# alexandre01/deepsvg

Measured on AMD Instinct MI355X. Metric: SVG icons/sec (train step) hierarchical_ordered d=256, higher is better.
Workload: dtype bf16; 1 GPU; hierarchical_ordered (Hierarchical, use_vae=False) G=8 S=30 d_model=256 ff=512 H=8 L=4x4; full train step = forward + SVGLoss + backward + grad-clip 1.0 + AdamW; dropout 0.1; global_batch=512, batch_per_gpu=512, parallelism=dp1, hip_graph=True, encoder_layout=packed (valid tokens only, exact)

## Files before the change

### deepsvg_amd/csrc/ffn_bwd_gate.hip

```cpp
#include <stdlib.h>
#include "mfma_frag.h"
#include "../../include/dsvg.h"

namespace {

constexpr int GT = 64;
constexpr int W2_BYTES = 256 * 64 * 2;
constexpr int SLOT = (2 * 64 * 128 + 64 * 64) * 2;
constexpr int HP_OFF = 2 * 64 * 128 * 2;
constexpr int NSLOT = 4;
constexpr int W2_AT = (NSLOT - 1) * SLOT;
constexpr int LDS_BYTES = NSLOT * SLOT;
static_assert(LDS_BYTES <= 160 * 1024, "LDS budget of a CU");
static_assert(W2_BYTES <= SLOT, "the W2p image fits a slot");

__device__ __forceinline__ int sw256(int r) { return ((r & 3) << 2) | ((r >> 2) & 3); }
__device__ __forceinline__ int sw128(int r) { return ((r >> 1) & 1) << 2; }

__device__ __forceinline__ void dma5(const char* s0, const char* s1, const char* s2, const char* s3, const char* s4,
                                     uint32_t lds) {
    uint32_t keep;
    asm volatile(
        "s_mov_b32 %0, m0\n\t"
        "s_mov_b32 m0, %6\n\t"
        "s_nop 0\n\t"
        "global_load_lds_dwordx4 %1, off\n\t"
        "s_add_u32 m0, m0, 0x400\n\t"
        "s_nop 0\n\t"
        "global_load_lds_dwordx4 %2, off\n\t"
        "s_add_u32 m0, m0, 0x400\n\t"
        "s_nop 0\n\t"
        "global_load_lds_dwordx4 %3, off\n\t"
        "s_add_u32 m0, m0, 0x400\n\t"
        "s_nop 0\n\t"
        "global_load_lds_dwordx4 %4, off\n\t"
        "s_add_u32 m0, m0, 0x400\n\t"
        "s_nop 0\n\t"
        "global_load_lds_dwordx4 %5, off\n\t"
        "s_mov_b32 m0, %0"
        : "=&s"(keep)
        : "v"(s0), "v"(s1), "v"(s2), "v"(s3), "v"(s4), "s"(lds)
        : "memory", "scc");
}
__device__ __forceinline__ void dma4(const char* s0, const char* s1, const char* s2, const char* s3, uint32_t lds) {
    uint32_t keep;
    asm volatile(
        "s_mov_b32 %0, m0\n\t"
        "s_mov_b32 m0, %5\n\t"
        "s_nop 0\n\t"
        "global_load_lds_dwordx4 %1, off\n\t"
        "s_add_u32 m0, m0, 0x400\n\t"
        "s_nop 0\n\t"
        "global_load_lds_dwordx4 %2, off\n\t"
        "s_add_u32 m0, m0, 0x400\n\t"
        "s_nop 0\n\t"
        "global_load_lds_dwordx4 %3, off\n\t"
        "s_add_u32 m0, m0, 0x400\n\t"
        "s_nop 0\n\t"
        "global_load_lds_dwordx4 %4, off\n\t"
        "s_mov_b32 m0, %0"
        : "=&s"(keep)
        : "v"(s0), "v"(s1), "v"(s2), "v"(s3), "s"(lds)
        : "memory", "scc");
}

__device__ __forceinline__ bf16x8 ld_tr(const char* img, uint32_t off0, uint32_t off1) {
    Frag8 f;
    f.h[0] = __builtin_amdgcn_ds_read_tr16_b64_v4i16((shortx4 __attribute__((address_space(3)))*)(img + off0));
    f.h[1] = __builtin_amdgcn_ds_read_tr16_b64_v4i16((shortx4 __attribute__((address_space(3)))*)(img + off1));
    return f.v;
}

__device__ __forceinline__ bf16x8 zero_from(const bf16x8& v, int lim) {
    Frag8 f;
    f.v = v;
    uint32_t w[4] = {f.u.x, f.u.y, f.u.z, f.u.w};
#pragma unroll
    for (int e = 0; e < 4; ++e) w[e] = 2 * e >= lim ? 0u : (2 * e + 1 >= lim ? (w[e] & 0xffffu) : w[e]);
    f.u = make_uint4(w[0], w[1], w[2], w[3]);
    return f.v;
}

__device__ __forceinline__ float rowsum8(const bf16x8& f, float s) {
    typedef __bf16 bf16x2 __attribute__((ext_vector_type(2)));
    Frag8 t;
    t.v = f;
    const uint32_t w[4] = {t.u.x, t.u.y, t.u.z, t.u.w};
    const bf16x2 one = __builtin_bit_cast(bf16x2, 0x3f803f80u);
#pragma unroll
    for (int e = 0; e < 4; ++e) s = __builtin_amdgcn_fdot2_f32_bf16(__builtin_bit_cast(bf16x2, w[e]), one, s, false);
    return s;
}

__global__ __launch_bounds__(512, 1) void ffn_gate_dw2_kernel(const bf16_t* __restrict__ dym, const bf16_t* __restrict__ hp,
                                                               const bf16_t* __restrict__ w2p, float gate_scale,
                                                               bf16_t* __restrict__ dpre, int T, int k_chunk, int xcd_map,
                                                               float* __restrict__ part, int part_bf16) {
    extern __shared__ __attribute__((aligned(1024))) char lds[];
    const int bid = (int)blockIdx.x;
    int c, z;
    if (xcd_map) { const int local = bid >> 3; c = local & 7; z = (local >> 3) * 8 + (bid & 7); }
    else { c = bid & 7; z = bid >> 3; }
    const int row_begin = z * k_chunk;
    const int row_end = min(T, row_begin + k_chunk);
    const int n_tiles = row_end > row_begin ? (row_end - row_begin + GT - 1) / GT : 0;

    const int tid = threadIdx.x, lane = tid & 63;
    const int wave = __builtin_amdgcn_readfirstlane(tid >> 6);
    const int h = lane >> 5;
    const uint32_t lds0 = (uint32_t)(uintptr_t)DSVG_LDS_PTR(lds);

    const char* src[5];
    int srow[5];
    long long sld[5];
#pragma unroll
    for (int i = 0; i < 5; ++i) {
        const int P = wave * 5 + i;
        if (P < 32) {
            const int r = 4 * (P & 15) + (lane >> 4);
            const int ch = (lane & 15) ^ sw256(r);
            src[i] = (const char*)dym + (size_t)(128 * (P >> 4) + 8 * ch) * 2;
            srow[i] = r;
            sld[i] = 256 * 2;
        } else {
            const int r = 8 * (P - 32) + (lane >> 3);
            const int ch = (lane & 7) ^ sw128(r);
            src[i] = (const char*)hp + (size_t)(64 * c + 8 * ch) * 2;
            srow[i] = r;
            sld[i] = 512 * 2;
        }
    }
    auto issue = [&](int s) {
        const int r0 = row_begin + s * GT;
        const char* a[5];
#pragma unroll
        for (int i = 0; i < 5; ++i) a[i] = src[i] + (size_t)min(r0 + srow[i], T - 1) * sld[i];
        const uint32_t dst = __builtin_amdgcn_readfirstlane(lds0 + (uint32_t)(s % NSLOT) * SLOT + (uint32_t)wave * 5 * 1024);
        dma5(a[0], a[1], a[2], a[3], a[4], dst);
    };
    auto wait_tile = [&](int s) {
        const int ahead = min(NSLOT - 2, n_tiles - 1 - s);
        if (ahead >= 2) asm volatile("s_waitcnt vmcnt(10)" ::: "memory");
        else if (ahead == 1) asm volatile("s_waitcnt vmcnt(5)" ::: "memory");
        else asm volatile("s_waitcnt vmcnt(0)" ::: "memory");
    };
    static_assert(NSLOT == 4, "wait_tile counts for a 4-slot ring");

    const int g = lane >> 4, q = lane & 15, qq = q >> 2, pp = q & 3;
    const bool p1 = wave < 4;
    const int wm = (wave >> 1) & 1, wn = wave & 1;
    const int ww = wave & 3;
    const int trow = 8 * (g >> 1) + qq;
    const int pr = 32 * wm + (lane & 31);
    const uint32_t w2_off = (uint32_t)(trow * 128 + 16 * ((4 * wn + 2 * (g & 1) + (pp >> 1)) ^ sw128(trow)) + 8 * (pp & 1));
    uint32_t da_off[2][2], hb_off[2];
#pragma unroll
    for (int it = 0; it < 2; ++it)
#pragma unroll
        for (int sc = 0; sc < 2; ++sc) {
            const int r = trow + 4 * sc;
            const int ch = 8 * (ww & 1) + 4 * it + 2 * (g & 1) + (pp >> 1);
            da_off[it][sc] = (uint32_t)((ww >> 1) * 16384 + r * 256 + 16 * (ch ^ sw256(r)) + 8 * (pp & 1));
        }
#pragma unroll
    for (int jn = 0; jn < 2; ++jn)
        hb_off[jn] = (uint32_t)(HP_OFF + trow * 128 + 16 * ((4 * jn + 2 * (g & 1) + (pp >> 1)) ^ sw128(trow)) + 8 * (pp & 1));

    floatx16 acc00, acc01, acc10, acc11;
#pragma unroll
    for (int r = 0; r < 16; ++r) { acc00[r] = 0.f; acc01[r] = 0.f; acc10[r] = 0.f; acc11[r] = 0.f; }
    const bool do_rs = !p1 && c == 0;
    float rsa0 = 0.f, rsa1 = 0.f, rsb0 = 0.f, rsb1 = 0.f;

    Frag8 w2f[16];

    auto dpre_tile = [&](int s) {
        const char* slot = lds + (s % NSLOT) * SLOT;
        const int r0 = row_begin + s * GT;
        floatx16 acc;
#pragma unroll
        for (int r = 0; r < 16; ++r) acc[r] = 0.f;
#pragma unroll
        for (int kk = 0; kk < 16; ++kk) {
            Frag8 a;
            a.u = *reinterpret_cast<const uint4*>(slot + (kk >> 3) * 16384 + pr * 256 +
                                                  16 * ((2 * (kk & 7) + h) ^ sw256(pr)));
            acc = __builtin_amdgcn_mfma_f32_32x32x16_bf16(w2f[kk].v, a.v, acc, 0, 0, 0);
        }
        uint32_t x[4][4];
#pragma unroll
        for (int gq = 0; gq < 4; ++gq)
#pragma unroll
            for (int e = 0; e < 4; ++e) x[gq][e] = __float_as_uint(acc[4 * gq + e]);
#pragma unroll
        for (int e = 0; e < 4; ++e) {
            auto s01 = __builtin_amdgcn_permlane32_swap(x[0][e], x[1][e], false, false);
            auto s23 = __builtin_amdgcn_permlane32_swap(x[2][e], x[3][e], false, false);
            x[0][e] = s01[0]; x[1][e] = s01[1]; x[2][e] = s23[0]; x[3][e] = s23[1];
        }
#pragma unroll
        for (int e = 0; e < 4; ++e) {
            auto s02 = __builtin_amdgcn_permlane32_swap(x[0][e], x[2][e], false, false);
            auto s13 = __builtin_amdgcn_permlane32_swap(x[1][e], x[3][e], false, false);
            x[0][e] = s02[0]; x[2][e] = s02[1]; x[1][e] = s13[0]; x[3][e] = s13[1];
        }
        uint4 pk[2];
#pragma unroll
        for (int cb = 0; cb < 2; ++cb) {
            float v[8];
#pragma unroll
            for (int e = 0; e < 4; ++e) { v[e] = __uint_as_float(x[2 * cb][e]); v[4 + e] = __uint_as_float(x[2 * cb + 1][e]); }
            const uint4 gt = *reinterpret_cast<const uint4*>(slot + HP_OFF + pr * 128 +
                                                             16 * ((4 * wn + 2 * h + cb) ^ sw128(pr)));
            const uint32_t gw[4] = {gt.x, gt.y, gt.z, gt.w};
#pragma unroll
            for (int e = 0; e < 4; ++e) {
                const float g0 = __uint_as_float(gw[e] << 16), g1 = __uint_as_float(gw[e] & 0xffff0000u);
                v[2 * e] = g0 > 0.f ? v[2 * e] * gate_scale : 0.f;
                v[2 * e + 1] = g1 > 0.f ? v[2 * e + 1] * gate_scale : 0.f;
            }
            pk[cb] = make_uint4(f2bf_pk(v[0], v[1]), f2bf_pk(v[2], v[3]), f2bf_pk(v[4], v[5]), f2bf_pk(v[6], v[7]));
        }
        const int m = r0 + pr;
        if (m < row_end) {
            bf16_t* cp = dpre + (size_t)m * 512 + 64 * c + 32 * wn + 16 * h;
            *reinterpret_cast<uint4*>(cp) = pk[0];
            *reinterpret_cast<uint4*>(cp + 8) = pk[1];
        }
    };
    auto g2p_tile = [&](int s) {
        const char* slot = lds + (s % NSLOT) * SLOT;
        const int r0 = row_begin + s * GT;
        const bool ragged = r0 + GT > row_end;
#pragma unroll
        for (int kk = 0; kk < 4; ++kk) {
            bf16x8 a0 = ld_tr(slot, da_off[0][0] + kk * 4096, da_off[0][1] + kk * 4096);
            bf16x8 a1 = ld_tr(slot, da_off[1][0] + kk * 4096, da_off[1][1] + kk * 4096);
            const bf16x8 b0 = ld_tr(slot, hb_off[0] + kk * 2048, hb_off[0] + kk * 2048 + 512);
            const bf16x8 b1 = ld_tr(slot, hb_off[1] + kk * 2048, hb_off[1] + kk * 2048 + 512);
            if (ragged) {
                const int lim = row_end - (r0 + 16 * kk + 8 * h);
                a0 = zero_from(a0, lim);
                a1 = zero_from(a1, lim);
            }
            acc00 = __builtin_amdgcn_mfma_f32_32x32x16_bf16(b0, a0, acc00, 0, 0, 0);
            acc01 = __builtin_amdgcn_mfma_f32_32x32x16_bf16(b0, a1, acc01, 0, 0, 0);
            acc10 = __builtin_amdgcn_mfma_f32_32x32x16_bf16(b1, a0, acc10, 0, 0, 0);
            acc11 = __builtin_amdgcn_mfma_f32_32x32x16_bf16(b1, a1, acc11, 0, 0, 0);
            if (do_rs) {
                if (kk < 2) { rsa0 = rowsum8(a0, rsa0); rsa1 = rowsum8(a1, rsa1); }
                else { rsb0 = rowsum8(a0, rsb0); rsb1 = rowsum8(a1, rsb1); }
            }
        }
    };

    if (n_tiles > 0) {
        issue(0);
        const char* a[4];
#pragma unroll
        for (int i = 0; i < 4; ++i) {
            const int r = 8 * (wave * 4 + i) + (lane >> 3);
            const int ch = (lane & 7) ^ sw128(r);
            a[i] = (const char*)w2p + ((size_t)r * 512 + 64 * c + 8 * ch) * 2;
        }
        dma4(a[0], a[1], a[2], a[3], __builtin_amdgcn_readfirstlane(lds0 + W2_AT + (uint32_t)wave * 4 * 1024));
        for (int s = 1; s < NSLOT - 1 && s < n_tiles; ++s) issue(s);
        wait_tile(0);
        __builtin_amdgcn_s_barrier();
    }
    if (p1) {
        if (n_tiles > 0) {
#pragma unroll
            for (int kk = 0; kk < 16; ++kk) w2f[kk].v = ld_tr(lds + W2_AT, w2_off + kk * 2048, w2_off + kk * 2048 + 512);
            asm volatile("s_waitcnt lgkmcnt(0)" ::: "memory");
        }
        for (int s = 0; s < n_tiles; ++s) {
            wait_tile(s);
            __builtin_amdgcn_s_barrier();
            if (s + NSLOT - 1 < n_tiles) issue(s + NSLOT - 1);
            dpre_tile(s);
        }
        return;
    }
    for (int s = 0; s < n_tiles; ++s) {
        wait_tile(s);
        __builtin_amdgcn_s_barrier();
        if (s + NSLOT - 1 < n_tiles) issue(s + NSLOT - 1);
        g2p_tile(s);
    }

    const size_t slice = dsvg_splitk_slice(256, 512, true);
    float* my_part = part + (size_t)z * slice;
    const int mrow = 64 * ww + (lane & 31);
    const int ncol = 64 * c;
    auto put = [&](const floatx16& v, int jn, int im) {
        const int m = mrow + 32 * im;
#pragma unroll
        for (int gq = 0; gq < 4; ++gq) {
            const int n = ncol + 32 * jn + 8 * gq + 4 * h;
            *reinterpret_cast<float4*>(my_part + (size_t)m * 512 + n) = make_float4(v[4 * gq], v[4 * gq + 1], v[4 * gq + 2], v[4 * gq + 3]);
        }
    };
    auto put_bf16 = [&](const floatx16& v, int jn, int im) {
        const int m = mrow + 32 * im;
        bf16_t* base = reinterpret_cast<bf16_t*>(my_part);
#pragma unroll
        for (int gp = 0; gp < 2; ++gp) {
            const uint32_t a0 = f2bf_pk(v[8 * gp + 0], v[8 * gp + 1]), a1 = f2bf_pk(v[8 * gp + 2], v[8 * gp + 3]);
            const uint32_t b0 = f2bf_pk(v[8 * gp + 4], v[8 * gp + 5]), b1 = f2bf_pk(v[8 * gp + 6], v[8 * gp + 7]);
            auto s0 = __builtin_amdgcn_permlane32_swap(a0, b0, false, false);
            auto s1 = __builtin_amdgcn_permlane32_swap(a1, b1, false, false);
            const int n = ncol + 32 * jn + 16 * gp + 8 * h;
            *reinterpret_cast<uint4*>(base + (size_t)m * 512 + n) = make_uint4(s0[0], s1[0], s0[1], s1[1]);
        }
    };
    if (part_bf16) { put_bf16(acc00, 0, 0); put_bf16(acc01, 0, 1); put_bf16(acc10, 1, 0); put_bf16(acc11, 1, 1); }
    else { put(acc00, 0, 0); put(acc01, 0, 1); put(acc10, 1, 0); put(acc11, 1, 1); }
    if (do_rs) {
        rsa0 += __shfl_xor(rsa0, 32, 64);
        rsa1 += __shfl_xor(rsa1, 32, 64);
        rsb0 += __shfl_xor(rsb0, 32, 64);
        rsb1 += __shfl_xor(rsb1, 32, 64);
        if (h == 0) {
            float* rs = my_part + 256 * 512;
            rs[mrow] = rsa0 + rsb0;
            rs[mrow + 32] = rsa1 + rsb1;
        }
    }
}

}

extern "C" int dsvg_ffn_gate_dw2(const void* dym, const void* hp, const void* w2p, float gate_scale, void* dpre,
                                 int64_t rows, int32_t split_k, float* g2p, float* db2, float* workspace,
                                 int64_t workspace_bytes, void* stream) {
    DSVG_CHECK_ARG(dym && hp && w2p && dpre && g2p && db2 && workspace, "ffn_gate_dw2: null operand");
    DSVG_CHECK_ARG(rows > 0 && rows < (1ll << 30) && split_k > 1, "ffn_gate_dw2: bad rows %lld / split_k %d",
                   (long long)rows, split_k);
    DSVG_CHECK_ARG(workspace_bytes >= dsvg_gemm_workspace_bytes(256, 512, split_k), "ffn_gate_dw2: workspace too small");
    DSVG_CHECK_ARG(!(((uintptr_t)dym | (uintptr_t)hp | (uintptr_t)w2p | (uintptr_t)dpre | (uintptr_t)workspace) & 15),
                   "ffn_gate_dw2: operands must be 16-byte aligned");
    static const bool pbf_on = !(getenv("DSVG_SPLITK_BF16") && atoi(getenv("DSVG_SPLITK_BF16")) == 0);
    hipStream_t st = (hipStream_t)stream;
    const int T = (int)rows;
    const int k_chunk = ((T + split_k - 1) / split_k + 63) / 64 * 64;
    int nsplit = (T + k_chunk - 1) / k_chunk;
    if ((split_k % 8) == 0) nsplit = split_k;
    const int pbf = (pbf_on && (T % 64) == 0) ? 1 : 0;
    static bool once = false;
    if (!once) {
        (void)hipFuncSetAttribute((const void*)ffn_gate_dw2_kernel, hipFuncAttributeMaxDynamicSharedMemorySize, LDS_BYTES);
        once = true;
    }
    hipLaunchKernelGGL(ffn_gate_dw2_kernel, dim3(8 * nsplit), dim3(512), LDS_BYTES, st, (const bf16_t*)dym,
                       (const bf16_t*)hp, (const bf16_t*)w2p, gate_scale, (bf16_t*)dpre, T, k_chunk,
                       (nsplit % 8) == 0 ? 1 : 0, workspace, pbf);
    DSVG_LAUNCH_CHECK("ffn_gate_dw2");
    const int64_t mn = 256 * 512;
    const int64_t slice = (int64_t)dsvg_splitk_slice(256, 512, true);
    int rc = pbf ? dsvg_reduce_partials_mixed(workspace, nsplit, slice, mn, mn, g2p, 0, st)
                 : dsvg_reduce_partials_strided(workspace, nsplit, slice, mn, g2p, 0, st);
    if (rc) return rc;
    return dsvg_reduce_partials_strided(workspace + mn, nsplit, slice, 256, db2, 0, st);
}
```

### deepsvg_amd/functional.py

```python
import math
import contextlib
import functools
import os

import torch

from . import ops

FFN_MIN_ROWS = int(os.environ.get("DSVG_FFN_MIN_ROWS", "16384"))
ATTN_MIN_ROWS = int(os.environ.get("DSVG_ATTN_MIN_ROWS", "16384"))
FFN_GATE_DW2 = os.environ.get("DSVG_FFN_GATE_DW2", "1") != "0"

LN_BWD_MASKED = os.environ.get("DSVG_LN_BWD_MASKED", "1") != "0"
DEFER_MORE = os.environ.get("DSVG_DEFER_MORE", "1") != "0"
HEAD_KPAD = os.environ.get("DSVG_HEAD_KPAD", "1") != "0"
GS_STACK = os.environ.get("DSVG_GS_STACK", "1") != "0"
_ATTN_VALU = os.environ.get("DSVG_ATTN_VALU") is not None
_ATTN_MFMA_MIN_S = int(os.environ.get("DSVG_ATTN_MFMA_MIN_S", "2"))
GS_REMAINDER = int(os.environ.get("DSVG_GS_REMAINDER", "512"))
SEQ_ROUND = 2048
HEAD_FUSED = os.environ.get("DSVG_HEAD_FUSED", "0") != "0"

_NULL_CTX = contextlib.nullcontext()

class Runtime:

    def __init__(self, dtype=torch.float32, seed=None, store=None, training=False, defer=False):
        self.dtype = dtype
        self.defer = bool(defer)
        self.seed = seed
        self.store = store
        self.training = training
        self.masked = {}
        self.last_layer_gs = False
        self.stack_group = None
        self.path_stage = False
        self.cond_grad = {}

    def cond_grad_block(self, z, rows):
        if z is None or z.dim() != 2 or z.stride(1) != 1 or z.dtype != torch.bfloat16:
            return None
        w, ld = z.shape[1], z.stride(0)
        if ld <= w or ld % w or w % 8 or w > 512:
            return None
        i = (z.storage_offset() % ld) // w
        if (z.storage_offset() % ld) % w:
            return None
        base = z.data_ptr() - i * w * z.element_size()
        key = (base, rows, ld)
        buf = self.cond_grad.get(key)
        if buf is None:
            if len(self.cond_grad) > 8:
                self.cond_grad.clear()
            buf = self.cond_grad[key] = torch.empty((rows, ld), dtype=z.dtype, device=z.device)
        return buf[:, i * w:(i + 1) * w]

    def deferring(self):
        return ops.DEFER if self.defer else _NULL_CTX

    def stack_group_begin(self):
        if self.stack_group is None:
            ops.GROUP.__enter__()
            self.stack_group = []
        return self.stack_group

    def stack_group_end(self):
        if self.stack_group is not None:
            ops.GROUP.__exit__(None, None, None)
            self.stack_group = None

    def deferring_tables(self):
        return ops.DEFER if self.defer and DEFER_MORE else _NULL_CTX

    def grouping(self):
        return ops.GROUP

    def p(self, rate):
        return float(rate) if (self.training and rate > 0.0) else 0.0

    def w(self, param):
        if self.dtype == torch.float32:
            return param.detach()
        if self.store is not None:
            v = self.store.lp(param)
            if v is not None:
                return v
        return param.detach().to(self.dtype)

    def grad_out(self, param):
        if self.store is not None:
            v = self.store.grad_view(param)
            if v is not None:
                return v
        return torch.empty(param.shape, dtype=torch.float32, device=param.device)


def _wgrad_tag():
    return ops.tag_default("wgrad") if ops.PROFILE_ON else _NULL_CTX


def _wgrad(rt, param, dy, x, *, a_drop_p=0.0, a_drop_site=0):
    out = rt.grad_out(param)
    n_out, k_in = param.shape
    T = dy.shape[0]
    with rt.deferring(), _wgrad_tag():
        ops.gemm(dy, x, a_kc=False, b_kc=False, out=out.view(n_out, k_in), a_drop_p=a_drop_p, a_drop_site=a_drop_site,
                 seed=rt.seed, split_k=ops.split_k_for(n_out, k_in, T))
    return out


def _wbgrad(rt, weight, bias, dy, x, blocks=None, *, out=None, split=None, defer=True):
    if split is None:
        split = ops.split_k_for(*weight.shape, dy.shape[0], target_blocks=blocks)
    dw, db = out if out is not None else (rt.grad_out(weight), rt.grad_out(bias))
    with (rt.deferring() if defer else _NULL_CTX), _wgrad_tag():
        if split > 1:
            ops.gemm(dy, x, a_kc=False, b_kc=False, out=dw, split_k=split, rowsum=db)
        else:
            ops.gemm(dy, x, a_kc=False, b_kc=False, out=dw)
            ops.colsum(dy, out=db)
    return dw, db


def _group_blocks(w):
    return 8 * -(-w.shape[0] // 128) * -(-w.shape[1] // 128)


def _bgrad(rt, param, dy, *, drop_p=0.0, drop_site=0):
    out = rt.grad_out(param)
    with rt.deferring():
        ops.colsum(dy, out=out, drop_p=drop_p, drop_site=drop_site, seed=rt.seed)
    return out


def _hand_masked(rt, dx, dxm, p, site):
    if len(rt.masked) > 8:
        rt.masked.clear()
    rt.masked[dx.data_ptr()] = (dxm, p, site, dx._version)


def _take_masked(rt, dx, p, site, rows=None):
    hit = rt.masked.pop(dx.data_ptr(), None)
    if hit is None:
        return None
    dxm, hp, hsite, ver = hit
    n = dx.shape[0] if rows is None else rows
    if (hp != p or hsite != site or dxm.dtype != dx.dtype or dxm.shape[0] < n or dxm.shape[1:] != dx.shape[1:]
            or dx._version != ver):
        return None
    return dxm[:n]


def _aligned2d(t, mult):
    if t.dim() == 2 and t.stride(1) == 1 and t.stride(0) % mult == 0 and t.data_ptr() % 16 == 0:
        return t
    rows, cols = t.shape
    ld = (cols + mult - 1) // mult * mult
    buf = torch.zeros((rows, ld), dtype=t.dtype, device=t.device)
    buf[:, :cols].copy_(t)
    return buf[:, :cols]


class LinearFn(torch.autograd.Function):

# ... 456 lines not shown
        if _gs_eligible(rt, x, key_mask, n_seq, S, n_heads) and not causal and seq_off is None and l is None and live is None:
            gs = rt.store.gs(win)
        if gs is not None:
            g = (z if wg is None else ops.gemm(z, rt.w(wg), bias=bg.detach())) if z is not None else None
            with ops.tag("gs"):
                res = ops.gs_layer_fwd(x, gs[0], bin_.detach(), bo.detach(), b1.detach(), b2.detach(), n1w.detach(),
                                       n1b.detach(), n2w.detach(), n2b.detach(), key_mask, n_seq, S, scale, 1e-5, p, site0,
                                       rt.seed, seq_add=g, train=want_bwd)
            if want_bwd:
                x2, mean1, rstd1, xn1, qkv, ao, x1, mean2, rstd2, xn2, h = res
            else:
                x2, mean1, rstd1, xn1, qkv, ao, x1, mean2, rstd2, xn2, h = (res,) + (None,) * 10
            ctx.gs, ctx.ffn_fused, ctx.tiles, ctx.causal, ctx.live = True, False, None, False, None
            rt.last_layer_gs = True
            ctx.rt, ctx.n_seq, ctx.S, ctx.n_heads, ctx.p, ctx.site0, ctx.scale = rt, n_seq, S, n_heads, p, site0, scale
            ctx.save_for_backward(x, key_mask, z, l, mean1, rstd1, xn1, qkv, ao, x1, mean2, rstd2, xn2, h,
                                  n1w, n1b, win, bin_, wo, bo, n2w, n2b, w1, b1, w2, b2, wg, bg, wg2, bg2, seq_off)
            return x2
        att = None
        if (_attn_fused_eligible(rt, x, x.shape[0], key_mask, n_heads, causal) and S <= 32
                and (seq_off is None or tiles is not None) and p <= 0.5):
            att = rt.store.attn(win)
        z_fused = False
        split = 0
        if (att is not None and want_bwd and GS_REMAINDER > 0 and seq_off is None and key_mask is None and l is None
                and x.shape[0] == n_seq * S and x.shape[0] >= FFN_MIN_ROWS and n_seq > SEQ_ROUND):
            rem = n_seq % SEQ_ROUND
            if 0 < rem <= GS_REMAINDER and rt.store.gs(win) is not None and rt.store.ffn(w1) is not None:
                split = n_seq - rem
        if split:
            gsr, ffn = rt.store.gs(win), rt.store.ffn(w1)
            T, R0 = x.shape[0], split * S
            bf = lambda w_: torch.empty((T, w_), dtype=x.dtype, device=x.device)
            f32 = lambda n_: torch.empty(n_, dtype=torch.float32, device=x.device)
            x1, xn1, qkv, ao, mean1, rstd1 = bf(256), bf(256), bf(768), bf(256), f32(T), f32(T)
            x2, h, xn2 = bf(256), bf(512), bf(256)
            g = None
            if z is not None:
                g = z if wg is None else ops.gemm(z, rt.w(wg), bias=bg.detach())
                z_fused = True
            with ops.tag("attn"):
                ops.attn_block_fwd(x[:R0], att, bin_.detach(), bo.detach(), n1w.detach(), n1b.detach(), None, split, S, scale,
                                   1e-5, p, site0, site0 + 1, rt.seed, train=True, seq_add=None if g is None else g[:split],
                                   site_seq_add=site0 + 2,
                                   into=(x1[:R0], xn1[:R0], qkv[:R0], ao[:R0], mean1[:R0], rstd1[:R0]))
            with ops.tag("ffn"):
                ops.ffn_fwd(x1[:R0], ffn[0], ffn[2], b2.detach(), 1e-5, p, site0 + 3, site0 + 4, rt.seed, out=x2[:R0],
                            train=True, into=(h[:R0], xn2[:R0]))
            with ops.tag("gs"):
                ops.gs_layer_fwd(x[R0:], gsr[0], bin_.detach(), bo.detach(), b1.detach(), b2.detach(), n1w.detach(),
                                 n1b.detach(), n2w.detach(), n2b.detach(), None, n_seq - split, S, scale, 1e-5, p, site0,
                                 rt.seed, seq_add=None if g is None else g[split:], train=True, seq_base=split, ffn_format=True,
                                 into=(x2[R0:], mean1[R0:], rstd1[R0:], xn1[R0:], qkv[R0:], ao[R0:], x1[R0:], f32(T - R0),
                                       f32(T - R0), xn2[R0:], h[R0:]))
            mean2 = rstd2 = None
        elif att is not None:
            g = None
            if z is not None and seq_off is None and x.shape[0] == n_seq * S:
                g = z if wg is None else ops.gemm(z, rt.w(wg), bias=bg.detach())
                z_fused = True
            with ops.tag("attn"):
                res = ops.attn_block_fwd(x, att, bin_.detach(), bo.detach(), n1w.detach(), n1b.detach(), key_mask, n_seq,
                                         S, scale, 1e-5, p, site0, site0 + 1, rt.seed, seq_off=seq_off, tiles=tiles,
                                         train=want_bwd, seq_add=g, site_seq_add=site0 + 2)
            if want_bwd:
                x1, xn1, qkv, ao, mean1, rstd1 = res
            else:
                x1, xn1, qkv, ao, mean1, rstd1 = res, None, None, None, None, None
        else:
            xn1, mean1, rstd1 = ops.layernorm_fwd(x, n1w.detach(), n1b.detach())
            qkv = ops.gemm(xn1, rt.w(win), bias=bin_.detach())
            if causal:
                ao = ops.attention_fwd(qkv, key_mask, n_seq, S, n_heads, scale, p, site0, rt.seed, causal=True)
            else:
                ao = ops.attention_fwd(qkv, key_mask, n_seq, S, n_heads, scale, p, site0, rt.seed, seq_off=seq_off,
                                       tiles=tiles, **_path_kw(rt, S))
            x1 = ops.gemm(ao, rt.w(wo), bias=bo.detach(), res=x, drop_p=p, drop_site=site0 + 1, seed=rt.seed)
        ctx.tiles, ctx.causal = tiles, causal
        if z is not None and not z_fused:
            g = z.contiguous() if wg is None else ops.gemm(z, rt.w(wg), bias=bg.detach())
            ops.bcast_add_fwd_(x1, g, n_seq, S, p, site0 + 2, rt.seed)
        if l is not None:
            g2 = ops.gemm(l, rt.w(wg2), bias=bg2.detach())
            ops.bcast_add_fwd_(x1, g2, n_seq, S, p, site0 + 5, rt.seed)
        ffn = rt.store.ffn(w1) if (rt.store is not None and x.dtype == torch.bfloat16 and x.shape[0] >= FFN_MIN_ROWS) else None
        ctx.ffn_fused = ffn is not None
        if split:
            pass
        elif ffn is not None:
            mean2 = rstd2 = None
            with ops.tag("ffn"):
                if want_bwd:
                    x2, h, xn2, _rstd = ops.ffn_fwd(x1, ffn[0], ffn[2], b2.detach(), 1e-5, p, site0 + 3, site0 + 4, rt.seed,
                                                    train=True)
                else:
                    xn2 = h = None
                    x2 = ops.ffn_fwd(x1, ffn[0], ffn[2], b2.detach(), 1e-5, p, site0 + 3, site0 + 4, rt.seed)
        else:
            with ops.tag("ffn"):
                xn2, mean2, rstd2 = ops.layernorm_fwd(x1, n2w.detach(), n2b.detach())
                h = ops.gemm(xn2, rt.w(w1), bias=b1.detach(), act=ops.RELU, drop_p=p, drop_site=site0 + 3, seed=rt.seed)
                x2 = ops.gemm(h, rt.w(w2), bias=b2.detach(), res=x1, drop_p=p, drop_site=site0 + 4, seed=rt.seed)
        ctx.rt, ctx.n_seq, ctx.S, ctx.n_heads, ctx.p, ctx.site0, ctx.scale = rt, n_seq, S, n_heads, p, site0, scale
        assert seq_off is None or (z is None and l is None), "packed layout: no per-sequence conditioning adds"
        ctx.live = _live_rows(live, x.shape[0])
        assert ctx.live is None or (seq_off is None and key_mask is None and l is None)
        ctx.save_for_backward(x, key_mask, z, l, mean1, rstd1, xn1, qkv, ao, x1, mean2, rstd2, xn2, h,
                              n1w, n1b, win, bin_, wo, bo, n2w, n2b, w1, b1, w2, b2, wg, bg, wg2, bg2, seq_off)
        return x2

    @staticmethod
    def backward(ctx, dx2):
        rt, n_seq, S, H, p, s0 = ctx.rt, ctx.n_seq, ctx.S, ctx.n_heads, ctx.p, ctx.site0
        (x, key_mask, z, l, mean1, rstd1, xn1, qkv, ao, x1, mean2, rstd2, xn2, h,
         n1w, n1b, win, bin_, wo, bo, n2w, n2b, w1, b1, w2, b2, wg, bg, wg2, bg2, seq_off) = ctx.saved_tensors
        dx2 = dx2.contiguous()
        full_rows, n_seq_full = x.shape[0], n_seq
        live = _armed(ctx.live)
        dx2_masked = _take_masked(rt, dx2, p, s0 + 4, rows=(live[1] if live is not None else None)) if p > 0 else None
        if live is not None:
            n_seq, R = live
            (dx2, x, mean1, rstd1, xn1, qkv, ao, x1, mean2, rstd2, xn2, h) = (
                (t[:R] if t is not None else None) for t in (dx2, x, mean1, rstd1, xn1, qkv, ao, x1, mean2, rstd2, xn2, h))
        inv_keep = ops.keep_scale(p)
        dx1m = None
        if ctx.gs:
            gs = rt.store.gs(win)
            with rt.deferring(), ops.tag("gs"):
                (dx, dx1, dym, dpre, dx1m, dqkv, dn2w, dn2b, dn1w, dn1b, *dg_) = ops.gs_layer_bwd(
                    dx2, gs[1], x, mean1, rstd1, qkv, x1, mean2, rstd2, h, n1w.detach(), n2w.detach(), key_mask, n_seq, S,
                    ctx.scale, p, s0, rt.seed, want_dx1=False, dgamma2=rt.grad_out(n2w),
                    dbeta2=rt.grad_out(n2b), dgamma1=rt.grad_out(n1w), dbeta1=rt.grad_out(n1b), want_dg=z is not None)
            dz = dg = None
            if z is not None:
                dg = dg_[0]
                if wg is None:
                    dz = dg
                elif ctx.needs_input_grad[3]:
                    dz = ops.gemm(dg, rt.w(wg), b_kc=False)
            (dw2, db2), (dw1, db1), (dwo, dbo), (dwin, dbin), (dwg, dbg) = _gs_queue_wgrads(
                rt, ctx.first_in_stack, (w2, b2, dym, h), (w1, b1, dpre, xn2), (wo, bo, dx1m, ao), (win, bin_, dqkv, xn1),
                cond=(wg if z is not None else None, bg, dg, z))
            return (None, dx, None, dz, None, None, None, None, None, None,
                    dn1w, dn1b, dwin, dbin, dwo, dbo, dn2w, dn2b, dw1, db1, dw2, db2, dwg, dbg, None, None, None, None, None,
                    None, None, None)
        if ctx.ffn_fused:
            pb, _b1f, w2p = rt.store.ffn(w1)[1:]
            T = x1.shape[0]
            with ops.tag("ffn"):
                g2p = torch.empty((256, 512), dtype=torch.float32, device=x1.device)
                g1p = torch.empty((512, 256), dtype=torch.float32, device=x1.device)
                db1p = torch.empty(512, dtype=torch.float32, device=x1.device)
                db2 = rt.grad_out(b2)
                s2, s1 = ops.split_k_for(256, 512, T), ops.split_k_for(512, 256, T)
                hp, xh = h, xn2
                dym = dx2_masked if dx2_masked is not None else ops.drop_apply(dx2, p, s0 + 4, rt.seed)
                if (FFN_GATE_DW2 and s2 > 1 and dym.is_cuda and dym.dtype == torch.bfloat16
                        and dym.is_contiguous() and hp.is_contiguous() and w2p.is_contiguous()):
                    with rt.deferring():
                        dpre = ops.ffn_gate_dw2(dym, hp, w2p, inv_keep, g2p, db2, s2)
                else:
                    _wbgrad(rt, None, None, dym, hp, out=(g2p, db2), split=s2)
                    dpre = ops.gemm(dym, w2p, b_kc=False, gate=hp, gate_scale=inv_keep)
                _wbgrad(rt, None, None, dpre, xh, out=(g1p, db1p), split=s1)
                dx1 = ops.ffn_bwd_dx(dpre, x1, dx2, pb)
                dw1, db1, dw2 = rt.grad_out(w1), rt.grad_out(b1), rt.grad_out(w2)
                dn2w, dn2b = rt.grad_out(n2w), rt.grad_out(n2b)
                fin = (g1p, db1p, g2p, w1.detach(), n2w.detach(), n2b.detach(), dw1.detach(), db1.detach(), dw2.detach(),
                       dn2w.detach(), dn2b.detach())
                if rt.defer:
                    ops.ffn_wgrad_finish_deferred(*fin)
                else:
                    ops.ffn_wgrad_finish(*fin)
            del hp, dpre, xh, dym
        else:
            with ops.tag("ffn"):
                dx2m = dx2_masked if dx2_masked is not None else ops.drop_apply(dx2, p, s0 + 4, rt.seed)
                dw2, db2 = _wbgrad(rt, w2, b2, dx2m, h)
                dh = ops.gemm(dx2m, rt.w(w2), b_kc=False, gate=h, gate_scale=inv_keep)
                dw1, db1 = _wbgrad(rt, w1, b1, dh, xn2)
                dxn2 = ops.gemm(dh, rt.w(w1), b_kc=False)
                with rt.deferring():
                    dx1, dn2w, dn2b = ops.layernorm_bwd(dxn2, x1, mean2, rstd2, n2w.detach(), res=dx2,
                                                        dgamma=rt.grad_out(n2w), dbeta=rt.grad_out(n2b))
            del dx2m
        dz = dl = dwg = dbg = dwg2 = dbg2 = None
        if l is not None:
            dg2 = ops.bcast_add_bwd(dx1, n_seq, S, p, s0 + 5, rt.seed)
            dwg2, dbg2 = _wbgrad(rt, wg2, bg2, dg2, l)
            if ctx.needs_input_grad[4]:
                dl = ops.gemm(dg2, rt.w(wg2), b_kc=False)
        if z is not None:
            vec = dx1.dtype == torch.bfloat16 and dx1.is_contiguous() and dx1.shape[1] % 8 == 0 and dx1.shape[1] <= 512
            dg_out = rt.cond_grad_block(z, n_seq_full) if (wg is None and vec and dx1.data_ptr() % 16 == 0) else None
            if p > 0 and vec and n_seq * S <= dx1.shape[0] <= n_seq_full * S:
                dg, dx1m = ops.bcast_add_bwd(dx1, n_seq, S, p, s0 + 2, rt.seed, n_seq_out=n_seq_full, mask_site=s0 + 1, out=dg_out)
            else:
                dg = ops.bcast_add_bwd(dx1, n_seq, S, p, s0 + 2, rt.seed, n_seq_out=n_seq_full, out=dg_out)
            if wg is None:
                dz = dg
            else:
                dwg, dbg = _wbgrad(rt, wg, bg, dg, z)
                if ctx.needs_input_grad[3]:
                    dz = ops.gemm(dg, rt.w(wg), b_kc=False)
        if dx1m is None:
            dx1m = ops.drop_apply(dx1, p, s0 + 1, rt.seed)
        dwo, dbo = _wbgrad(rt, wo, bo, dx1m, ao)
        wob = None
        if (not _ATTN_VALU and S >= _ATTN_MFMA_MIN_S and _attn_fused_eligible(rt, x, x.shape[0], key_mask, H, ctx.causal)
                and ((seq_off is None and 16 < S <= 32 and x.shape[0] >= n_seq * S) or (seq_off is not None and ctx.tiles is not None))):
            wob = rt.store.attn_bwd(win)
        if wob is not None:
            dqkv = ops.attention_bwd_outproj(qkv, key_mask, dx1m, wob, n_seq, S, ctx.scale, p, s0, rt.seed, seq_off=seq_off,
                                             tiles=ctx.tiles)
        else:
            dao = ops.gemm(dx1m, rt.w(wo), b_kc=False)
            if ctx.causal:
                dqkv = ops.attention_bwd(qkv, key_mask, dao, n_seq, S, H, ctx.scale, p, s0, rt.seed, causal=True)
            else:
                dqkv = ops.attention_bwd(qkv, key_mask, dao, n_seq, S, H, ctx.scale, p, s0, rt.seed, seq_off=seq_off,
                                         tiles=ctx.tiles, **_path_kw(rt, S))
        del dx1m
        dwin, dbin = _wbgrad(rt, win, bin_, dqkv, xn1)
        dx_out = None
        if live is not None:
            dx_full = torch.empty((full_rows, x.shape[1]), dtype=x.dtype, device=x.device)
            dx_out = dx_full[:x.shape[0]]
        mk = (p, ctx.mask_below, rt.seed) if (ctx.mask_below is not None and p > 0) else None
        with rt.deferring():
            dxn1 = ops.gemm(dqkv, rt.w(win), b_kc=False)
            out = ops.layernorm_bwd(dxn1, x, mean1, rstd1, n1w.detach(), res=dx1, dx=dx_out,
                                    dgamma=rt.grad_out(n1w), dbeta=rt.grad_out(n1b), masked=mk)
            dx, dn1w, dn1b = out[:3]
        if live is not None:
            dx = dx_full
        if mk is not None:
            _hand_masked(rt, dx, out[3], p, ctx.mask_below)
        return (None, dx, None, dz, dl, None, None, None, None, None,
                dn1w, dn1b, dwin, dbin, dwo, dbo, dn2w, dn2b, dw1, db1, dw2, db2, dwg, dbg, dwg2, dbg2, None, None, None,
                None, None, None)


def gs_stack_eligible(rt, x, key_mask, n_seq, S, n_heads, n_layers, wins):
    return (GS_STACK and x.dim() == 2 and _gs_eligible(rt, x, key_mask, n_seq, S, n_heads)
            and 1 <= n_layers <= ops.GS_STACK_MAX and all(rt.store.gs(w) is not None for w in wins))


class GsStackFn(torch.autograd.Function):

    @staticmethod
    def forward(ctx, rt, x, key_mask, n_seq, S, n_heads, drop_rate, site0, n_layers, has_g, *tensors):
        p = rt.p(drop_rate)
        per = 13 if has_g else 12
        assert len(tensors) == per * n_layers
        scale = float(x.shape[1] // n_heads) ** -0.5
        want_bwd = any(ctx.needs_input_grad)
        layers = []
        for i in range(n_layers):
            n1w, n1b, win, bin_, wo, bo, n2w, n2b, w1, b1, w2, b2 = tensors[per * i:per * i + 12]
            layers.append(dict(img=rt.store.gs(win)[0], in_bias=bin_.detach(), out_bias=bo.detach(), b1=b1.detach(), b2=b2.detach(),
                               gamma1=n1w.detach(), beta1=n1b.detach(), gamma2=n2w.detach(), beta2=n2b.detach(),
                               site0=site0 + 8 * i, seq_add=tensors[per * i + 12] if has_g else None))
        with ops.tag("gs"):
            res = ops.gs_stack_fwd(x, layers, key_mask, n_seq, S, scale, 1e-5, p, rt.seed, train=want_bwd)
        rt.last_layer_gs = True
        ctx.rt, ctx.n_seq, ctx.S, ctx.p, ctx.site0, ctx.scale, ctx.n, ctx.has_g = rt, n_seq, S, p, site0, scale, n_layers, has_g
        if not want_bwd:
            return res[-1]
        saved = [x, key_mask]
        for r in res:
            saved += list(r)
        ctx.save_for_backward(*saved, *tensors)
        return res[-1][0]

    @staticmethod
    def backward(ctx, dx2):
        rt, n_seq, S, p, n, has_g = ctx.rt, ctx.n_seq, ctx.S, ctx.p, ctx.n, ctx.has_g
        sv = ctx.saved_tensors
        x, key_mask = sv[0], sv[1]
        acts = [sv[2 + 11 * i:2 + 11 * (i + 1)] for i in range(n)]
        tensors = sv[2 + 11 * n:]
        per = 13 if has_g else 12
        prm = [tensors[per * i:per * i + 12] for i in range(n)]
        layers = []
        for i in range(n):
            x2, mean1, rstd1, xn1, qkv, ao, x1, mean2, rstd2, xn2, h = acts[i]
            n1w, n1b, win, bin_, wo, bo, n2w, n2b, w1, b1, w2, b2 = prm[i]
            layers.append(dict(img=rt.store.gs(win)[1], x=x if i == 0 else acts[i - 1][0], mean1=mean1, rstd1=rstd1, qkv=qkv, x1=x1,
                               mean2=mean2, rstd2=rstd2, h=h, gamma1=n1w.detach(), gamma2=n2w.detach(), site0=ctx.site0 + 8 * i,
                               dgamma2=rt.grad_out(n2w), dbeta2=rt.grad_out(n2b), dgamma1=rt.grad_out(n1w),
                               dbeta1=rt.grad_out(n1b)))
        with rt.deferring(), ops.tag("gs"):
            dx, ops_, dgcat = ops.gs_stack_bwd(dx2.contiguous(), layers, key_mask, n_seq, S, ctx.scale, p, rt.seed, want_dg=has_g)
        grads = [None] * (per * n)
        for i in range(n - 1, -1, -1):
            x2, mean1, rstd1, xn1, qkv, ao, x1, mean2, rstd2, xn2, h = acts[i]
            n1w, n1b, win, bin_, wo, bo, n2w, n2b, w1, b1, w2, b2 = prm[i]
            dym, dpre, dx1m, dqkv = ops_[i]
            (dw2, db2), (dw1, db1), (dwo, dbo), (dwin, dbin), _ = _gs_queue_wgrads(
                rt, i == 0, (w2, b2, dym, h), (w1, b1, dpre, xn2), (wo, bo, dx1m, ao), (win, bin_, dqkv, xn1))
            L = layers[i]
            grads[per * i:per * i + 12] = [L["dgamma1"], L["dbeta1"], dwin, dbin, dwo, dbo, L["dgamma2"], L["dbeta2"], dw1, db1, dw2, db2]
            if has_g:
                grads[per * i + 12] = dgcat[:, 256 * i:256 * (i + 1)]
        return (None, dx, None, None, None, None, None, None, None, None, *grads)


# ... 153 lines not shown
```

Baseline: 92040 icons/s.

## Widen gate/dW2 kernel column tile to 128 and double split-k

The fused FFN backward gate plus dW2 kernel now gives each block 128 hidden columns instead of 64, so only 4 column blocks are launched per k-chunk. It holds a larger W2 image that spans two LDS slots and uses a 3-slot ring with 6 DMA pieces per wave. The dpre path issues two MFMAs per loaded W2 fragment, and the dW2 path keeps 8 accumulators. This cuts redundant reloads of dym across column blocks and raises MFMA work per LDS byte. To keep the grid occupied, the split-k count targets twice as many blocks. The cost is a shallower prefetch pipeline, more registers, more partials to reduce, and an extra barrier before the second tile can be issued.

```diff
diff --git a/deepsvg_amd/csrc/ffn_bwd_gate.hip b/deepsvg_amd/csrc/ffn_bwd_gate.hip
--- a/deepsvg_amd/csrc/ffn_bwd_gate.hip
+++ b/deepsvg_amd/csrc/ffn_bwd_gate.hip
@@ -5,24 +5,26 @@
 namespace {
 
 constexpr int GT = 64;
-constexpr int W2_BYTES = 256 * 64 * 2;
-constexpr int SLOT = (2 * 64 * 128 + 64 * 64) * 2;
-constexpr int HP_OFF = 2 * 64 * 128 * 2;
-constexpr int NSLOT = 4;
-constexpr int W2_AT = (NSLOT - 1) * SLOT;
+constexpr int IMG = 64 * 128 * 2;
+constexpr int W2_BYTES = 4 * IMG;
+constexpr int SLOT = 3 * IMG;
+constexpr int HP_OFF = 2 * IMG;
+constexpr int NSLOT = 3;
+constexpr int PIECES = SLOT / 1024 / 8;
+constexpr int W2_AT = SLOT;
 constexpr int LDS_BYTES = NSLOT * SLOT;
 static_assert(LDS_BYTES <= 160 * 1024, "LDS budget of a CU");
-static_assert(W2_BYTES <= SLOT, "the W2p image fits a slot");
+static_assert(W2_AT + W2_BYTES <= LDS_BYTES, "the W2p image fits slots 1-2");
+static_assert(PIECES == 6, "dma6 / wait_tile count 6 pieces per wave and tile");
 
 __device__ __forceinline__ int sw256(int r) { return ((r & 3) << 2) | ((r >> 2) & 3); }
-__device__ __forceinline__ int sw128(int r) { return ((r >> 1) & 1) << 2; }
-
-__device__ __forceinline__ void dma5(const char* s0, const char* s1, const char* s2, const char* s3, const char* s4,
-                                     uint32_t lds) {
+
+__device__ __forceinline__ void dma6(const char* s0, const char* s1, const char* s2, const char* s3, const char* s4,
+                                     const char* s5, uint32_t lds) {
     uint32_t keep;
     asm volatile(
         "s_mov_b32 %0, m0\n\t"
-        "s_mov_b32 m0, %6\n\t"
+        "s_mov_b32 m0, %7\n\t"
         "s_nop 0\n\t"
         "global_load_lds_dwordx4 %1, off\n\t"
         "s_add_u32 m0, m0, 0x400\n\t"
@@ -37,9 +39,12 @@
         "s_add_u32 m0, m0, 0x400\n\t"
         "s_nop 0\n\t"
         "global_load_lds_dwordx4 %5, off\n\t"
+        "s_add_u32 m0, m0, 0x400\n\t"
+        "s_nop 0\n\t"
+        "global_load_lds_dwordx4 %6, off\n\t"
         "s_mov_b32 m0, %0"
         : "=&s"(keep)
-        : "v"(s0), "v"(s1), "v"(s2), "v"(s3), "v"(s4), "s"(lds)
+        : "v"(s0), "v"(s1), "v"(s2), "v"(s3), "v"(s4), "v"(s5), "s"(lds)
         : "memory", "scc");
 }
 __device__ __forceinline__ void dma4(const char* s0, const char* s1, const char* s2, const char* s3, uint32_t lds) {
@@ -99,8 +104,8 @@
     extern __shared__ __attribute__((aligned(1024))) char lds[];
     const int bid = (int)blockIdx.x;
     int c, z;
-    if (xcd_map) { const int local = bid >> 3; c = local & 7; z = (local >> 3) * 8 + (bid & 7); }
-    else { c = bid & 7; z = bid >> 3; }
+    if (xcd_map) { const int local = bid >> 3; c = local & 3; z = (local >> 2) * 8 + (bid & 7); }
+    else { c = bid & 3; z = bid >> 2; }
     const int row_begin = z * k_chunk;
     const int row_end = min(T, row_begin + k_chunk);
     const int n_tiles = row_end > row_begin ? (row_end - row_begin + GT - 1) / GT : 0;
@@ -110,88 +115,75 @@
     const int h = lane >> 5;
     const uint32_t lds0 = (uint32_t)(uintptr_t)DSVG_LDS_PTR(lds);
 
-    const char* src[5];
-    int srow[5];
-    long long sld[5];
-#pragma unroll
-    for (int i = 0; i < 5; ++i) {
-        const int P = wave * 5 + i;
+    const char* src[PIECES];
+    int srow[PIECES];
+    long long sld[PIECES];
+#pragma unroll
+    for (int i = 0; i < PIECES; ++i) {
+        const int P = wave * PIECES + i;
+        const int r = 4 * (P & 15) + (lane >> 4);
+        const int ch = (lane & 15) ^ sw256(r);
+        srow[i] = r;
         if (P < 32) {
-            const int r = 4 * (P & 15) + (lane >> 4);
-            const int ch = (lane & 15) ^ sw256(r);
             src[i] = (const char*)dym + (size_t)(128 * (P >> 4) + 8 * ch) * 2;
-            srow[i] = r;
             sld[i] = 256 * 2;
         } else {
-            const int r = 8 * (P - 32) + (lane >> 3);
-            const int ch = (lane & 7) ^ sw128(r);
-            src[i] = (const char*)hp + (size_t)(64 * c + 8 * ch) * 2;
-            srow[i] = r;
+            src[i] = (const char*)hp + (size_t)(128 * c + 8 * ch) * 2;
             sld[i] = 512 * 2;
         }
     }
     auto issue = [&](int s) {
         const int r0 = row_begin + s * GT;
-        const char* a[5];
-#pragma unroll
-        for (int i = 0; i < 5; ++i) a[i] = src[i] + (size_t)min(r0 + srow[i], T - 1) * sld[i];
-        const uint32_t dst = __builtin_amdgcn_readfirstlane(lds0 + (uint32_t)(s % NSLOT) * SLOT + (uint32_t)wave * 5 * 1024);
-        dma5(a[0], a[1], a[2], a[3], a[4], dst);
+        const char* a[PIECES];
+#pragma unroll
+        for (int i = 0; i < PIECES; ++i) a[i] = src[i] + (size_t)min(r0 + srow[i], T - 1) * sld[i];
+        const uint32_t dst =
+            __builtin_amdgcn_readfirstlane(lds0 + (uint32_t)(s % NSLOT) * SLOT + (uint32_t)wave * PIECES * 1024);
+        dma6(a[0], a[1], a[2], a[3], a[4], a[5], dst);
     };
     auto wait_tile = [&](int s) {
-        const int ahead = min(NSLOT - 2, n_tiles - 1 - s);
-        if (ahead >= 2) asm volatile("s_waitcnt vmcnt(10)" ::: "memory");
-        else if (ahead == 1) asm volatile("s_waitcnt vmcnt(5)" ::: "memory");
+        if (s + 1 < n_tiles) asm volatile("s_waitcnt vmcnt(6)" ::: "memory");
         else asm volatile("s_waitcnt vmcnt(0)" ::: "memory");
     };
-    static_assert(NSLOT == 4, "wait_tile counts for a 4-slot ring");
+    static_assert(NSLOT == 3, "wait_tile counts for a 3-slot ring");
 
     const int g = lane >> 4, q = lane & 15, qq = q >> 2, pp = q & 3;
     const bool p1 = wave < 4;
-    const int wm = (wave >> 1) & 1, wn = wave & 1;
     const int ww = wave & 3;
     const int trow = 8 * (g >> 1) + qq;
-    const int pr = 32 * wm + (lane & 31);
-    const uint32_t w2_off = (uint32_t)(trow * 128 + 16 * ((4 * wn + 2 * (g & 1) + (pp >> 1)) ^ sw128(trow)) + 8 * (pp & 1));
-    uint32_t da_off[2][2], hb_off[2];
-#pragma unroll
-    for (int it = 0; it < 2; ++it)
-#pragma unroll
-        for (int sc = 0; sc < 2; ++sc) {
-            const int r = trow + 4 * sc;
-            const int ch = 8 * (ww & 1) + 4 * it + 2 * (g & 1) + (pp >> 1);
-            da_off[it][sc] = (uint32_t)((ww >> 1) * 16384 + r * 256 + 16 * (ch ^ sw256(r)) + 8 * (pp & 1));
-        }
-#pragma unroll
-    for (int jn = 0; jn < 2; ++jn)
-        hb_off[jn] = (uint32_t)(HP_OFF + trow * 128 + 16 * ((4 * jn + 2 * (g & 1) + (pp >> 1)) ^ sw128(trow)) + 8 * (pp & 1));
-
-    floatx16 acc00, acc01, acc10, acc11;
-#pragma unroll
-    for (int r = 0; r < 16; ++r) { acc00[r] = 0.f; acc01[r] = 0.f; acc10[r] = 0.f; acc11[r] = 0.f; }
+    auto tr_off = [&](int grp, int sc) {
+        const int r = trow + 4 * sc;
+        return (uint32_t)(r * 256 + 16 * ((4 * grp + 2 * (g & 1) + (pp >> 1)) ^ sw256(r)) + 8 * (pp & 1));
+    };
+    const int pr = lane & 31;
+    const uint32_t w2_off[2] = {W2_AT + tr_off(ww, 0), W2_AT + tr_off(ww, 1)};
+    uint32_t da_off[2][2], hb_off[4][2];
+#pragma unroll
+    for (int sc = 0; sc < 2; ++sc) {
+#pragma unroll
+        for (int it = 0; it < 2; ++it) da_off[it][sc] = (uint32_t)((ww >> 1) * IMG) + tr_off(2 * (ww & 1) + it, sc);
+#pragma unroll
+        for (int jn = 0; jn < 4; ++jn) hb_off[jn][sc] = (uint32_t)HP_OFF + tr_off(jn, sc);
+    }
+
+    floatx16 acc[4][2];
+#pragma unroll
+    for (int jn = 0; jn < 4; ++jn)
+#pragma unroll
+        for (int it = 0; it < 2; ++it)
+#pragma unroll
+            for (int r = 0; r < 16; ++r) acc[jn][it][r] = 0.f;
     const bool do_rs = !p1 && c == 0;
     float rsa0 = 0.f, rsa1 = 0.f, rsb0 = 0.f, rsb1 = 0.f;
 
     Frag8 w2f[16];
 
-    auto dpre_tile = [&](int s) {
-        const char* slot = lds + (s % NSLOT) * SLOT;
-        const int r0 = row_begin + s * GT;
-        floatx16 acc;
-#pragma unroll
-        for (int r = 0; r < 16; ++r) acc[r] = 0.f;
-#pragma unroll
-        for (int kk = 0; kk < 16; ++kk) {
-            Frag8 a;
-            a.u = *reinterpret_cast<const uint4*>(slot + (kk >> 3) * 16384 + pr * 256 +
-                                                  16 * ((2 * (kk & 7) + h) ^ sw256(pr)));
-            acc = __builtin_amdgcn_mfma_f32_32x32x16_bf16(w2f[kk].v, a.v, acc, 0, 0, 0);
-        }
+    auto dpre_store = [&](const floatx16& dacc, const char* slot, int trw, int m) {
         uint32_t x[4][4];
 #pragma unroll
         for (int gq = 0; gq < 4; ++gq)
 #pragma unroll
-            for (int e = 0; e < 4; ++e) x[gq][e] = __float_as_uint(acc[4 * gq + e]);
+            for (int e = 0; e < 4; ++e) x[gq][e] = __float_as_uint(dacc[4 * gq + e]);
 #pragma unroll
         for (int e = 0; e < 4; ++e) {
             auto s01 = __builtin_amdgcn_permlane32_swap(x[0][e], x[1][e], false, false);
@@ -210,8 +202,8 @@
             float v[8];
 #pragma unroll
             for (int e = 0; e < 4; ++e) { v[e] = __uint_as_float(x[2 * cb][e]); v[4 + e] = __uint_as_float(x[2 * cb + 1][e]); }
-            const uint4 gt = *reinterpret_cast<const uint4*>(slot + HP_OFF + pr * 128 +
-                                                             16 * ((4 * wn + 2 * h + cb) ^ sw128(pr)));
+            const uint4 gt = *reinterpret_cast<const uint4*>(slot + HP_OFF + trw * 256 +
+                                                             16 * ((4 * ww + 2 * h + cb) ^ sw256(trw)));
             const uint32_t gw[4] = {gt.x, gt.y, gt.z, gt.w};
 #pragma unroll
             for (int e = 0; e < 4; ++e) {
@@ -221,12 +213,29 @@
             }
             pk[cb] = make_uint4(f2bf_pk(v[0], v[1]), f2bf_pk(v[2], v[3]), f2bf_pk(v[4], v[5]), f2bf_pk(v[6], v[7]));
         }
-        const int m = r0 + pr;
         if (m < row_end) {
-            bf16_t* cp = dpre + (size_t)m * 512 + 64 * c + 32 * wn + 16 * h;
+            bf16_t* cp = dpre + (size_t)m * 512 + 128 * c + 32 * ww + 16 * h;
             *reinterpret_cast<uint4*>(cp) = pk[0];
             *reinterpret_cast<uint4*>(cp + 8) = pk[1];
         }
+    };
+    auto dpre_tile = [&](int s) {
+        const char* slot = lds + (s % NSLOT) * SLOT;
+        const int r0 = row_begin + s * GT;
+        floatx16 d0, d1;
+#pragma unroll
+        for (int r = 0; r < 16; ++r) { d0[r] = 0.f; d1[r] = 0.f; }
+#pragma unroll
+        for (int kk = 0; kk < 16; ++kk) {
+            const char* rowp = slot + (kk >> 3) * IMG + pr * 256 + 16 * ((2 * (kk & 7) + h) ^ sw256(pr));
+            Frag8 a0, a1;
+            a0.u = *reinterpret_cast<const uint4*>(rowp);
+            a1.u = *reinterpret_cast<const uint4*>(rowp + 32 * 256);
+            d0 = __builtin_amdgcn_mfma_f32_32x32x16_bf16(w2f[kk].v, a0.v, d0, 0, 0, 0);
+            d1 = __builtin_amdgcn_mfma_f32_32x32x16_bf16(w2f[kk].v, a1.v, d1, 0, 0, 0);
+        }
+        dpre_store(d0, slot, pr, r0 + pr);
+        dpre_store(d1, slot, 32 + pr, r0 + 32 + pr);
     };
     auto g2p_tile = [&](int s) {
         const char* slot = lds + (s % NSLOT) * SLOT;
@@ -236,17 +245,17 @@
         for (int kk = 0; kk < 4; ++kk) {
             bf16x8 a0 = ld_tr(slot, da_off[0][0] + kk * 4096, da_off[0][1] + kk * 4096);
             bf16x8 a1 = ld_tr(slot, da_off[1][0] + kk * 4096, da_off[1][1] + kk * 4096);
-            const bf16x8 b0 = ld_tr(slot, hb_off[0] + kk * 2048, hb_off[0] + kk * 2048 + 512);
-            const bf16x8 b1 = ld_tr(slot, hb_off[1] + kk * 2048, hb_off[1] + kk * 2048 + 512);
             if (ragged) {
                 const int lim = row_end - (r0 + 16 * kk + 8 * h);
                 a0 = zero_from(a0, lim);
                 a1 = zero_from(a1, lim);
             }
-            acc00 = __builtin_amdgcn_mfma_f32_32x32x16_bf16(b0, a0, acc00, 0, 0, 0);
-            acc01 = __builtin_amdgcn_mfma_f32_32x32x16_bf16(b0, a1, acc01, 0, 0, 0);
-            acc10 = __builtin_amdgcn_mfma_f32_32x32x16_bf16(b1, a0, acc10, 0, 0, 0);
-            acc11 = __builtin_amdgcn_mfma_f32_32x32x16_bf16(b1, a1, acc11, 0, 0, 0);
+#pragma unroll
+            for (int jn = 0; jn < 4; ++jn) {
+                const bf16x8 b = ld_tr(slot, hb_off[jn][0] + kk * 4096, hb_off[jn][1] + kk * 4096);
+                acc[jn][0] = __builtin_amdgcn_mfma_f32_32x32x16_bf16(b, a0, acc[jn][0], 0, 0, 0);
+                acc[jn][1] = __builtin_amdgcn_mfma_f32_32x32x16_bf16(b, a1, acc[jn][1], 0, 0, 0);
+            }
             if (do_rs) {
                 if (kk < 2) { rsa0 = rowsum8(a0, rsa0); rsa1 = rowsum8(a1, rsa1); }
                 else { rsb0 = rowsum8(a0, rsb0); rsb1 = rowsum8(a1, rsb1); }
@@ -256,23 +265,26 @@
 
     if (n_tiles > 0) {
         issue(0);
-        const char* a[4];
-#pragma unroll
-        for (int i = 0; i < 4; ++i) {
-            const int r = 8 * (wave * 4 + i) + (lane >> 3);
-            const int ch = (lane & 7) ^ sw128(r);
-            a[i] = (const char*)w2p + ((size_t)r * 512 + 64 * c + 8 * ch) * 2;
-        }
-        dma4(a[0], a[1], a[2], a[3], __builtin_amdgcn_readfirstlane(lds0 + W2_AT + (uint32_t)wave * 4 * 1024));
-        for (int s = 1; s < NSLOT - 1 && s < n_tiles; ++s) issue(s);
-        wait_tile(0);
+        const char* a[8];
+#pragma unroll
+        for (int i = 0; i < 8; ++i) {
+            const int r = 4 * (wave * 8 + i) + (lane >> 4);
+            const int ch = (lane & 15) ^ sw256(r);
+            a[i] = (const char*)w2p + ((size_t)r * 512 + 128 * c + 8 * ch) * 2;
+        }
+        const uint32_t dst = __builtin_amdgcn_readfirstlane(lds0 + W2_AT + (uint32_t)wave * 8 * 1024);
+        dma4(a[0], a[1], a[2], a[3], dst);
+        dma4(a[4], a[5], a[6], a[7], dst + 4 * 1024);
+        asm volatile("s_waitcnt vmcnt(0)" ::: "memory");
         __builtin_amdgcn_s_barrier();
     }
     if (p1) {
         if (n_tiles > 0) {
 #pragma unroll
-            for (int kk = 0; kk < 16; ++kk) w2f[kk].v = ld_tr(lds + W2_AT, w2_off + kk * 2048, w2_off + kk * 2048 + 512);
+            for (int kk = 0; kk < 16; ++kk) w2f[kk].v = ld_tr(lds, w2_off[0] + kk * 4096, w2_off[1] + kk * 4096);
             asm volatile("s_waitcnt lgkmcnt(0)" ::: "memory");
+            __builtin_amdgcn_s_barrier();
+            if (n_tiles > 1) issue(1);
         }
         for (int s = 0; s < n_tiles; ++s) {
             wait_tile(s);
@@ -282,6 +294,10 @@
         }
         return;
     }
+    if (n_tiles > 0) {
+        __builtin_amdgcn_s_barrier();
+        if (n_tiles > 1) issue(1);
+    }
     for (int s = 0; s < n_tiles; ++s) {
         wait_tile(s);
         __builtin_amdgcn_s_barrier();
@@ -292,7 +308,7 @@
     const size_t slice = dsvg_splitk_slice(256, 512, true);
     float* my_part = part + (size_t)z * slice;
     const int mrow = 64 * ww + (lane & 31);
-    const int ncol = 64 * c;
+    const int ncol = 128 * c;
     auto put = [&](const floatx16& v, int jn, int im) {
         const int m = mrow + 32 * im;
 #pragma unroll
@@ -314,8 +330,13 @@
             *reinterpret_cast<uint4*>(base + (size_t)m * 512 + n) = make_uint4(s0[0], s1[0], s0[1], s1[1]);
         }
     };
-    if (part_bf16) { put_bf16(acc00, 0, 0); put_bf16(acc01, 0, 1); put_bf16(acc10, 1, 0); put_bf16(acc11, 1, 1); }
-    else { put(acc00, 0, 0); put(acc01, 0, 1); put(acc10, 1, 0); put(acc11, 1, 1); }
+#pragma unroll
+    for (int jn = 0; jn < 4; ++jn)
+#pragma unroll
+        for (int it = 0; it < 2; ++it) {
+            if (part_bf16) put_bf16(acc[jn][it], jn, it);
+            else put(acc[jn][it], jn, it);
+        }
     if (do_rs) {
         rsa0 += __shfl_xor(rsa0, 32, 64);
         rsa1 += __shfl_xor(rsa1, 32, 64);
@@ -352,7 +373,7 @@
         (void)hipFuncSetAttribute((const void*)ffn_gate_dw2_kernel, hipFuncAttributeMaxDynamicSharedMemorySize, LDS_BYTES);
         once = true;
     }
-    hipLaunchKernelGGL(ffn_gate_dw2_kernel, dim3(8 * nsplit), dim3(512), LDS_BYTES, st, (const bf16_t*)dym,
+    hipLaunchKernelGGL(ffn_gate_dw2_kernel, dim3(4 * nsplit), dim3(512), LDS_BYTES, st, (const bf16_t*)dym,
                        (const bf16_t*)hp, (const bf16_t*)w2p, gate_scale, (bf16_t*)dpre, T, k_chunk,
                        (nsplit % 8) == 0 ? 1 : 0, workspace, pbf);
     DSVG_LAUNCH_CHECK("ffn_gate_dw2");
diff --git a/deepsvg_amd/functional.py b/deepsvg_amd/functional.py
--- a/deepsvg_amd/functional.py
+++ b/deepsvg_amd/functional.py
@@ -10,6 +10,12 @@
 FFN_MIN_ROWS = int(os.environ.get("DSVG_FFN_MIN_ROWS", "16384"))
 ATTN_MIN_ROWS = int(os.environ.get("DSVG_ATTN_MIN_ROWS", "16384"))
 FFN_GATE_DW2 = os.environ.get("DSVG_FFN_GATE_DW2", "1") != "0"
+FFN_GATE_DW2_SPLIT = int(os.environ.get("DSVG_FFN_GATE_DW2_SPLIT", "0"))
+
+
+def gate_dw2_split(T):
+    return FFN_GATE_DW2_SPLIT or ops.split_k_for(256, 512, T, target_blocks=2 * ops._SPLITK_BLOCKS)
+
 
 LN_BWD_MASKED = os.environ.get("DSVG_LN_BWD_MASKED", "1") != "0"
 DEFER_MORE = os.environ.get("DSVG_DEFER_MORE", "1") != "0"
@@ -772,7 +778,7 @@
                 g1p = torch.empty((512, 256), dtype=torch.float32, device=x1.device)
                 db1p = torch.empty(512, dtype=torch.float32, device=x1.device)
                 db2 = rt.grad_out(b2)
-                s2, s1 = ops.split_k_for(256, 512, T), ops.split_k_for(512, 256, T)
+                s2, s1 = gate_dw2_split(T), ops.split_k_for(512, 256, T)
                 hp, xh = h, xn2
                 dym = dx2_masked if dx2_masked is not None else ops.drop_apply(dx2, p, s0 + 4, rt.seed)
                 if (FFN_GATE_DW2 and s2 > 1 and dym.is_cuda and dym.dtype == torch.bfloat16
```

Result: no change. 92010 icons/s (-0.0%).
